# brendisurfs/Distributed-Backtesting-Exploration

Hardware: AMD Instinct MI355X
Metric: bar-evals/sec (symbols x params x bars) (higher is better)
Workload: dtype f64+int64; 1 GPU; BASELINE config 2: SMA fast/slow crossover, 5,000 symbols x 2,520 daily bars x 400 params per GPU; symbols_total=5000, symbols_per_gpu=5000, bars=2520, params=400, topk=100, parallelism=dp1 (contiguous symbol shards; exchange: none)

## Files before the change

### distributed-backtesting-exploration_amd/csrc/device_common.h

```cpp
#pragma once
#include <type_traits>

#include "internal.h"

namespace bt {

__host__ __device__ inline uint64_t trade_mix(uint64_t w) {
    const uint64_t z = (w ^ (w >> 29)) * 0xBF58476D1CE4E5B9ULL;
    return z ^ (z >> 32);
}
__host__ __device__ inline uint64_t trade_mix_et(uint32_t e, uint32_t t, bool lg) {
    const uint32_t lo = e ^ (t << 2) ^ (t << 31);
    const uint32_t hi = (t >> 1) ^ (lg ? 0x40000002u : 0u);
    const uint64_t z = (((uint64_t)hi << 32) | lo) * 0xBF58476D1CE4E5B9ULL;
    return z ^ (z >> 32);
}
constexpr int kDstLevels = 6;
constexpr int kKeyStride = kTile + 1;

typedef __int128 i128;
typedef __attribute__((address_space(3))) double lds_f64;

struct __attribute__((aligned(16))) Agg {
    int32_t mx, mn, dd, du;
// ... 22 lines not shown
}

__device__ __forceinline__ Agg dst_query(const Agg* D, const int32_t* cT, int a, int b) {
    if (a == b) return agg_one(cT[a]);
    const int r = dst_row(a, b);
    return agg_merge(D[r * kTile + a], D[r * kTile + b]);
}

__device__ __forceinline__ Agg dst_query_bf(const Agg* D, int a, int b) {
    const Agg* Dr = dst_rowp(D, a, b);
    return agg_merge(Dr[a], Dr[b]);
}

__device__ __forceinline__ Agg dst_query_w(const Agg* D, int a, int b) {
    const Agg* Dr = dst_rowp(D, a, b);
    const int4 u = *reinterpret_cast<const int4*>(Dr + a);
    const int4 v = *reinterpret_cast<const int4*>(Dr + b);
    asm volatile("" ::"v"(u.x), "v"(u.y), "v"(u.z), "v"(u.w), "v"(v.x), "v"(v.y), "v"(v.z), "v"(v.w));
    return agg_merge(Agg{u.x, u.y, u.z, u.w}, Agg{v.x, v.y, v.z, v.w});
}

constexpr Agg kAggId = {0, 0x7FFFFFFF, 0, 0};

__device__ __forceinline__ int64_t wave_iscan_i64(int64_t x) {
    uint32_t lo = (uint32_t)x, hi = (uint32_t)((uint64_t)x >> 32);
#define BT_DPP_STEP(ctrl, rmask)                                                      \
    {                                                                                 \
        const uint32_t ylo = __builtin_amdgcn_update_dpp(0u, lo, ctrl, rmask, 0xf, false); \
        const uint32_t yhi = __builtin_amdgcn_update_dpp(0u, hi, ctrl, rmask, 0xf, false); \
        const uint64_t r = (((uint64_t)hi << 32) | lo) + (((uint64_t)yhi << 32) | ylo);   \
        lo = (uint32_t)r;                                                             \
        hi = (uint32_t)(r >> 32);                                                     \
    }
    BT_DPP_STEP(0x111, 0xf)
    BT_DPP_STEP(0x112, 0xf)
    BT_DPP_STEP(0x114, 0xf)
    BT_DPP_STEP(0x118, 0xf)
    BT_DPP_STEP(0x142, 0xa)
    BT_DPP_STEP(0x143, 0xc)
#undef BT_DPP_STEP
    return (int64_t)(((uint64_t)hi << 32) | lo);
}

#define BT_S64_CTRLS(X)                                                                   \
    X("row_shr:1 row_mask:0xf bank_mask:0xf bound_ctrl:1")                                \
    X("row_shr:2 row_mask:0xf bank_mask:0xf bound_ctrl:1")                                \
    X("row_shr:4 row_mask:0xf bank_mask:0xf bound_ctrl:1")                                \
    X("row_shr:8 row_mask:0xf bank_mask:0xf bound_ctrl:1")                                \
    X("row_bcast:15 row_mask:0xa bank_mask:0xf")                                          \
    X("row_bcast:31 row_mask:0xc bank_mask:0xf")
__device__ __forceinline__ int64_t wave_iscan_i64_ac(int64_t x) {
    uint32_t lo = (uint32_t)x, hi = (uint32_t)((uint64_t)x >> 32);
#define BT_S64_ONE(ctrl)                                                                   \
    "s_nop 1\n"                                                                            \
    "v_add_co_u32_dpp %0, vcc, %0, %0 " ctrl "\n"                                          \
    "v_addc_co_u32_dpp %1, vcc, %1, %1, vcc " ctrl "\n"
    asm volatile(BT_S64_CTRLS(BT_S64_ONE) "s_nop 1" : "+v"(lo), "+v"(hi) : : "vcc");
#undef BT_S64_ONE
    return (int64_t)(((uint64_t)hi << 32) | lo);
}
__device__ __forceinline__ void wave_iscan2_i64_ac(int64_t& x, int64_t& y) {
    uint32_t xl = (uint32_t)x, xh = (uint32_t)((uint64_t)x >> 32);
    uint32_t yl = (uint32_t)y, yh = (uint32_t)((uint64_t)y >> 32);
#define BT_S64_TWO(ctrl)                                                                   \
    "v_add_co_u32_dpp %0, vcc, %0, %0 " ctrl "\n"                                          \
    "v_addc_co_u32_dpp %1, vcc, %1, %1, vcc " ctrl "\n"                                    \
    "v_add_co_u32_dpp %2, vcc, %2, %2 " ctrl "\n"                                          \
    "v_addc_co_u32_dpp %3, vcc, %3, %3, vcc " ctrl "\n"
    asm volatile("s_nop 1\n" BT_S64_CTRLS(BT_S64_TWO) "s_nop 1"
                 : "+v"(xl), "+v"(xh), "+v"(yl), "+v"(yh) : : "vcc");
#undef BT_S64_TWO
    x = (int64_t)(((uint64_t)xh << 32) | xl);
    y = (int64_t)(((uint64_t)yh << 32) | yl);
}
#undef BT_S64_CTRLS

__device__ __forceinline__ uint32_t wave_iscan_u32(uint32_t x) {
    x += __builtin_amdgcn_update_dpp(0u, x, 0x111, 0xf, 0xf, false);
    x += __builtin_amdgcn_update_dpp(0u, x, 0x112, 0xf, 0xf, false);
    x += __builtin_amdgcn_update_dpp(0u, x, 0x114, 0xf, 0xf, false);
    x += __builtin_amdgcn_update_dpp(0u, x, 0x118, 0xf, 0xf, false);
    x += __builtin_amdgcn_update_dpp(0u, x, 0x142, 0xa, 0xf, false);
    x += __builtin_amdgcn_update_dpp(0u, x, 0x143, 0xc, 0xf, false);
    return x;
}

template <int CTRL>
__device__ __forceinline__ int32_t dpp(int32_t old, int32_t x) {
    int32_t r = (int32_t)__builtin_amdgcn_update_dpp((uint32_t)old, (uint32_t)x, CTRL, 0xf, 0xf, false);
    asm volatile("" : "+v"(r));
    return r;
}

template <int M>
__device__ __forceinline__ int32_t dst_partner(int32_t x, int lane) {
    if constexpr (M == 1) {
        return dpp<0xB1>(0, x);
    } else if constexpr (M == 2) {
        return dpp<0x0F>(0, x);
    } else if constexpr (M == 3) {
        const int32_t hm = dpp<0x141>(0, x);
        const int32_t q3 = dpp<0xFF>(0, hm), q0 = dpp<0x00>(0, hm);
        return (lane & 4) ? q3 : q0;
    } else if constexpr (M == 4) {
        const int32_t r0 = dpp<0x150>(0, x), r15 = dpp<0x15F>(0, x);
        return (lane & 8) ? r0 : r15;
    } else {
        static_assert(M == 5, "six levels for 64-lane tiles");
        const int32_t l0 = (int32_t)__builtin_amdgcn_readlane((uint32_t)x, 0);
        const int32_t l31 = (int32_t)__builtin_amdgcn_readlane((uint32_t)x, 31);
        const int32_t l32 = (int32_t)__builtin_amdgcn_readlane((uint32_t)x, 32);
        const int32_t l63 = (int32_t)__builtin_amdgcn_readlane((uint32_t)x, 63);
        return (lane & 16) ? ((lane & 32) ? l32 : l0) : ((lane & 32) ? l63 : l31);
    }
}

template <int M, bool LDSX = false>
__device__ __forceinline__ Agg dst_partner_agg(const Agg& a, int lane) {
    if constexpr (LDSX && M >= 3) {
        constexpr int half = 1 << (M - 1), grp = 1 << M;
        const int src = (lane & half) ? (lane & ~(grp - 1)) : (lane | (grp - 1));
        return Agg{__builtin_amdgcn_ds_bpermute(src << 2, a.mx), __builtin_amdgcn_ds_bpermute(src << 2, a.mn),
                   __builtin_amdgcn_ds_bpermute(src << 2, a.dd), __builtin_amdgcn_ds_bpermute(src << 2, a.du)};
    }
    return Agg{dst_partner<M>(a.mx, lane), dst_partner<M>(a.mn, lane), dst_partner<M>(a.dd, lane),
               dst_partner<M>(a.du, lane)};
}

template <bool LDSX = false>
__device__ __forceinline__ void dst_build(int32_t c, int lane, Agg* D) {
    if (LDSX) asm volatile("" : "+v"(lane));
    Agg S = agg_one(c), Pp = S;
    D[(kDstLevels - 1) * kTile + lane] = S;
    auto level = [&](auto mtag) {
        constexpr int m = decltype(mtag)::value;
        const bool left = (lane & (1 << (m - 1))) == 0;
        const Agg part = dst_partner_agg<m, LDSX>(agg_sel(left, S, Pp), lane);
        S = agg_sel(left, agg_merge(S, part), S);
        Pp = agg_sel(left, Pp, agg_merge(part, Pp));
        D[(kDstLevels - 1 - m) * kTile + lane] = agg_sel(((lane >> m) & 1) != 0, Pp, S);
    };
    level(std::integral_constant<int, 1>{});
    level(std::integral_constant<int, 2>{});
    level(std::integral_constant<int, 3>{});
    level(std::integral_constant<int, 4>{});
    level(std::integral_constant<int, 5>{});
    static_assert(kDstLevels == 6, "levels 1..5 above");
}

__device__ __forceinline__ int64_t lane63_i64(int64_t x) {
    const uint32_t lo = __builtin_amdgcn_readlane((uint32_t)x, 63);
    const uint32_t hi = __builtin_amdgcn_readlane((uint32_t)((uint64_t)x >> 32), 63);
    return (int64_t)(((uint64_t)hi << 32) | lo);
}

__device__ __forceinline__ void fixed_ret(int32_t c, int32_t cp, int64_t& q, int64_t& q2) {
    const double ret = (double)((int64_t)c - cp) / (double)cp;
    q = (int64_t)rint(ret * 72057594037927936.0);
    const double rr = ret * ret;
    q2 = (int64_t)rint(rr * 72057594037927936.0);
}

__device__ __forceinline__ void wave_add_trades(const Out& out, int ntr) {
    unsigned long long v = (unsigned long long)ntr;
#pragma unroll
    for (int d = 32; d > 0; d >>= 1) v += __shfl_down(v, d, 64);
// ... 5 lines not shown
```

### distributed-backtesting-exploration_amd/csrc/engine.cpp

```cpp
#include <algorithm>
#include <cmath>
#include <cstdio>
#include <cstdlib>
#include <cstring>
#include <memory>
#include <string>
#include <vector>

#include "batch.h"
#include "csv.h"
#include "engine_state.h"
#include "topk_rules.h"

using namespace bt;

static thread_local std::string g_err;

void bt::set_last_error(const std::string& s) { g_err = s; }

namespace {

const char* kernel_name(int32_t strategy) {
    switch (strategy) {
        case BT_SMA_CROSS: return "bt::sma_kernel";
        case BT_EMA_OLS: return "bt::ema_tile_kernel";
        default: return "bt::boll_tile_kernel";
    }
}

std::string validate_and_copy(bt_engine* e, const bt_config& c) {
    const std::string err = plan_grid(c, e->grid);
    if (!err.empty()) return err;
    AxisSpec ax[4];
    const int nax = config_axes(c, ax);
    for (int i = 0; i < nax; ++i) e->ax[i].assign(ax[i].v, ax[i].v + ax[i].n);
    e->P = e->grid.n_params;
    if (c.annualization <= 0) return "annualization must be positive";
    e->grid.sqrt_ann = std::sqrt((double)c.annualization);
    if (c.topk < 0 || c.topk > kTopkMax) return "topk must be in [0, 1024]";
    if ((c.flags & BT_FLAG_PARITY) && c.trade_cap <= 0) return "parity mode needs trade_cap > 0";
    return "";
}

void upload_grid(bt_engine* e) {
    const int32_t** dst[4] = {&e->grid.a, &e->grid.b, &e->grid.c, &e->grid.d};
    for (int i = 0; i < 4; ++i) {
        *dst[i] = nullptr;
        if (e->ax[i].empty()) continue;
        e->d_axes[i].ensure(e->ax[i].size());
        HIPCHK(hipMemcpy(e->d_axes[i].p, e->ax[i].data(), e->ax[i].size() * 4, hipMemcpyHostToDevice));
        *dst[i] = e->d_axes[i].p;
    }
    e->grid.kwin = nullptr;
    e->grid.krecip = nullptr;
    if (e->cfg.strategy == BT_SMA_CROSS) {
        std::vector<int32_t> win(e->ax[0]);
        win.insert(win.end(), e->ax[1].begin(), e->ax[1].end());
        win.resize((win.size() + kKeyGrab - 1) / kKeyGrab * kKeyGrab, 1);
        std::vector<double> recip(win.size());
        for (size_t i = 0; i < win.size(); ++i) recip[i] = key_recip(win[i]);
        e->d_kwin.ensure(win.size());
        e->d_krecip.ensure(win.size());
        HIPCHK(hipMemcpy(e->d_kwin.p, win.data(), win.size() * sizeof(int32_t), hipMemcpyHostToDevice));
        HIPCHK(hipMemcpy(e->d_krecip.p, recip.data(), recip.size() * sizeof(double), hipMemcpyHostToDevice));
        e->grid.kwin = e->d_kwin.p;
        e->grid.krecip = e->d_krecip.p;
    }
}

static_assert(kStageAlign == kRowAlign, "batch.h lays staging rows out as the device columns");

void set_dataset(bt_engine* e, std::vector<SymDesc>&& syms, int64_t rows) {
    sync_all(e);
    e->syms = std::move(syms);
    e->rows = rows;
    e->max_bars = 0;
    for (const SymDesc& sd : e->syms) e->max_bars = std::max(e->max_bars, sd.bars);
    const size_t n_sym = e->syms.size();
    e->d_syms.ensure(std::max<size_t>(1, n_sym));
    if (n_sym)
        HIPCHK(hipMemcpyAsync(e->d_syms.p, e->syms.data(), n_sym * sizeof(SymDesc),
                              hipMemcpyHostToDevice, e->stream));
    const size_t r = std::max<int64_t>(1, rows);
    e->d_c.ensure(r);
    if (has_hl(e)) {
        e->d_h.ensure(r);
        e->d_l.ensure(r);
    }
    e->ran = false;
}

void layout(bt_engine* e, int32_t n_sym, const int32_t* bars, const int64_t* ids) {
    std::vector<SymDesc> syms((size_t)n_sym);
    int64_t off = 0;
    for (int32_t s = 0; s < n_sym; ++s) {
        syms[s].off = off;
        syms[s].bars = bars[s];
        syms[s].id = (int32_t)ids[s];
        off += align_rows(bars[s]);
    }
    set_dataset(e, std::move(syms), off);
}

TopkWork topk_work(bt_engine* e) {
    return TopkWork{e->d_hist.p, e->d_state.p, e->d_counts.p, e->d_above.p, e->d_cand.p,
                    kTopkCap, e->d_top.p + 1, reinterpret_cast<int32_t*>(e->d_top.p)};
}

void ensure_outputs(bt_engine* e) {
    const size_t n = (size_t)e->syms.size() * e->P;
    for (int b = 0; b < 2; ++b) {
        e->d_sum[b].ensure(std::max<size_t>(1, n));
        e->d_key[b].ensure(std::max<size_t>(1, n));
    }
    e->d_ntr_ring.ensure(kNtrRing);
    if (e->cfg.flags & BT_FLAG_PARITY) {
        e->d_sums.ensure(std::max<size_t>(1, n));
        e->d_trades.ensure(std::max<size_t>(1, n * (size_t)e->cfg.trade_cap));
    }
    if (e->cfg.topk > 0 && !e->topk_ready) {
        e->d_hist.ensure(4096);
        e->d_counts.ensure(2);
        e->d_state.ensure(4);
        e->d_above.ensure(kTopkCap);
        e->d_cand.ensure(kTopkCap);
        e->d_top.ensure(kTopkMax + 1);
        e->h_top.ensure(kTopkMax + 1);
        HIPCHK(launch_topk_init(topk_work(e), e->stream));
        e->topk_ready = true;
    }
}

void run_impl(bt_engine* e) {
    activate(e);
    ensure_outputs(e);
    const int32_t S = (int32_t)e->syms.size();
    const int64_t run = e->nrun++;
    const int b = (int)(run & 1);
    e->cur = b;
    if (e->tdone_armed[b] && hipEventQuery(e->ev_tdone[b]) != hipSuccess)
        HIPCHK(hipStreamWaitEvent(e->stream, e->ev_tdone[b], 0));
    Out out{};
    out.sum = e->d_sum[b].p;
    out.key = e->d_key[b].p;
    const bool parity = (e->cfg.flags & BT_FLAG_PARITY) != 0;
// ... 559 lines not shown
```

### distributed-backtesting-exploration_amd/csrc/internal.h

```cpp
#pragma once
#include <hip/hip_runtime.h>
#include <stdint.h>

#include <string>

#include "../../include/bt.h"

#ifdef BT_PROFILING
#define BT_ABL(g, bit) (((g).ablate & (bit)) != 0)
#define BT_PRIO(g, shift, dflt) (BT_ABL(g, 1 << 20) ? (((g).ablate >> (shift)) & 3) : (dflt))
#else
#define BT_ABL(g, bit) false
#define BT_PRIO(g, shift, dflt) (dflt)
#endif
constexpr int kDbgSlots = 80, kDbgBlocks = 1024;

namespace bt {

constexpr int kTile = 64;
constexpr int kRowAlign = 64;

struct SymDesc {
    int64_t off;
    int32_t bars;
    int32_t id;
};

struct Grid {
    int32_t strategy;
    int32_t n_params;
    int32_t na, nb, nc, nd;
    int32_t band_bps, k_den;
    int32_t wmax;
    int32_t ring;
    double sqrt_ann;
    double kn2[8];
    int32_t kmin_idx;
    int32_t ablate;
    const int32_t* a;
    const int32_t* b;
    const int32_t* c;
    const int32_t* d;
    const int32_t* kwin;
    const double* krecip;
};
constexpr int kKeyGrab = 4;

struct Out {
    bt_summary* sum;
    uint64_t* key;
    bt_sums* sums;
    bt_trade* trades;
    int32_t trade_cap;
    unsigned long long* n_trades;
    unsigned long long* dbg;
};

struct SegRec {
    int32_t ntr, expo;
    int32_t start_pos, start_e;
    int32_t end_pos, end_e, end_ce, pad;
    int32_t end_agg[4];
    int64_t R;
    int64_t A, B, C, D;
    uint64_t h;
    uint64_t s1lo;
    int64_t s1hi;
    uint64_t s2lo;
    int64_t s2hi;
};
static_assert(sizeof(SegRec) == 128, "SegRec layout");
struct SmaSegRec {
    int32_t ntr;
    int32_t e0;
    int32_t start_pos, end_pos;
    int32_t end_e, end_ce;
    int32_t x1, px1;
    int32_t agg1[4];
    int32_t end_agg[4];
    int64_t R;
    int64_t B, C, D;
    uint64_t h;
    uint64_t s1lo, s2lo;
    int32_t s1hi, s2hi;
};
static_assert(sizeof(SmaSegRec) == sizeof(SegRec), "SmaSegRec is one 128-B SegRec slot");
struct SegArgs {
    SegRec* rec;
    int8_t* pos;
    unsigned long long* refixed;
    double* ema;
    int32_t G;
    int32_t burn_tiles;
};
constexpr int kEmaSegStride = 128;
struct LaunchPlan;
hipError_t launch_gen(const SymDesc* syms, int32_t n_sym, uint64_t seed, int32_t freq,
                      int32_t* o, int32_t* h, int32_t* l, int32_t* c, hipStream_t st);
hipError_t launch_sma(const SymDesc* syms, int32_t n_sym, const int32_t* close, const Grid& g,
                      const Out& out, bool parity, const SegArgs& seg, const LaunchPlan& pl,
                      hipStream_t st);
hipError_t launch_ema_ols(const SymDesc* syms, int32_t n_sym, const int32_t* close, const Grid& g,
                          const Out& out, bool parity, const SegArgs& seg, const LaunchPlan& pl,
                          hipStream_t st);
hipError_t launch_boll(const SymDesc* syms, int32_t n_sym, const int32_t* high, const int32_t* low,
                       const int32_t* close, const Grid& g, const Out& out, bool parity,
                       const SegArgs& seg, const LaunchPlan& pl, hipStream_t st);

struct ReplayLane {
    int64_t off;
    int32_t bars;
    int32_t param;
};
struct ReplayOut {
    bt_summary* sum;
    bt_trade* trades;
    int32_t trade_cap;
    int64_t* equity;
    int8_t* pos;
    int64_t pitch;
};
hipError_t launch_replay(const ReplayLane* lanes, int32_t n, const int32_t* high, const int32_t* low,
                         const int32_t* close, const Grid& g, const ReplayOut& o, hipStream_t st);

struct WfArgs {
    const SymDesc* syms;
    const int32_t* bounds;
    bt_fold* rec;
    bt_wf_step* steps;
    int32_t n_rows, P, K;
    int32_t train, j0, n_steps;
};
struct WalkfwdPlan;
hipError_t launch_wf_walk(const WfArgs& a, const int32_t* high, const int32_t* low, const int32_t* close,
                          const Grid& g, hipStream_t st);
hipError_t launch_wf_select(const WfArgs& a, const Grid& g, const WalkfwdPlan& pl, hipStream_t st);

struct PfLane {
    int64_t off;
    int32_t bars;
    int32_t param;
    int32_t from, to;
};
static_assert(sizeof(PfLane) == 24, "PfLane layout");
struct PfWork {
    unsigned long long* acc_pnl;
    unsigned long long* acc_cnt;
    int64_t pitch;
    int32_t R;
    int32_t T;
    int32_t n_lanes, lo, hi;
    int64_t* pnl;
    int64_t* equity;
    int32_t* n_long;
    int32_t* n_short;
    bt_pf_summary* sum;
};
struct PortfolioPlan;
hipError_t launch_portfolio(const PfLane* lanes, int32_t n, const int32_t* high, const int32_t* low,
                            const int32_t* close, const Grid& g, const PfWork& w, const PortfolioPlan& pl,
                            hipStream_t st);

struct SurfacePlan;
struct SurfaceWork {
    bt_param_agg* partial;
    bt_param_agg* fold;
    bt_topk_rec* best_partial;
    bt_param_agg* agg;
    bt_topk_rec* best;
};
hipError_t launch_surface(const bt_summary* sum, const int32_t* ids, int32_t id_stride, int32_t S,
                          int32_t P, const SurfacePlan& pl, const SurfaceWork& w, hipStream_t st);

constexpr int kTopkCap = 2048;
constexpr int kTopkMax = 1024;
struct TopkWork {
    unsigned int* hist;
    unsigned long long* state;
    unsigned int* counts;
    unsigned long long* above;
    unsigned long long* cand;
    int cap;
    bt_topk_rec* out;
    int32_t* out_n;
};
hipError_t launch_topk(const uint64_t* key, const bt_summary* sum, const SymDesc* syms,
                       int64_t n, int32_t P, int32_t k, const TopkWork& w, hipStream_t st, bool lds_free_hist = false);
hipError_t launch_topk_init(const TopkWork& w, hipStream_t st);

void set_last_error(const std::string& s);
inline bool topk_less(const bt_topk_rec& a, const bt_topk_rec& b);
struct ExchangeView {
    hipStream_t tstream;
    int32_t device, topk;
    const bt_topk_rec* d_top;
    const unsigned long long* d_ntr;
    int64_t bar_evals;
};
bool engine_exchange_view(bt_engine* e, ExchangeView& v, std::string& err);
void engine_exchange_enqueued(bt_engine* e);

__host__ __device__ inline double key_recip(int W) { return (1.0 / (double)W) * (1.0 + 0x1p-47); }

__host__ __device__ inline uint64_t order_key(double x) {
    union { double d; uint64_t u; } v;
    v.d = x;
    return (v.u >> 63) ? ~v.u : (v.u | 0x8000000000000000ULL);
}

__host__ __device__ inline double i128_to_double(uint64_t lo, int64_t hi) {
    const bool neg = hi < 0;
    uint64_t mh = (uint64_t)hi, ml = lo;
    if (neg) {
        ml = ~ml + 1;
        mh = ~mh + (ml == 0 ? 1 : 0);
    }
    if (mh == 0 && ml == 0) return 0.0;
    int lz = mh ? __builtin_clzll(mh) : 64 + __builtin_clzll(ml);
    uint64_t nh, nl;
    if (lz >= 64) {
        nh = ml << (lz - 64);
        nl = 0;
    } else if (lz == 0) {
        nh = mh;
        nl = ml;
    } else {
        nh = (mh << lz) | (ml >> (64 - lz));
        nl = ml << lz;
    }
    uint64_t mant = nh >> 11;
    const uint64_t rem_hi = nh & 0x7FFULL;
    const uint64_t half = 0x400ULL;
    bool up;
    if (rem_hi > half) up = true;
    else if (rem_hi < half) up = false;
    else up = (nl != 0) || (mant & 1);
    mant += up ? 1 : 0;
    double r = (double)mant;
#ifdef __HIP_DEVICE_COMPILE__
    r = ldexp(r, 75 - lz);
#else
    r = __builtin_ldexp(r, 75 - lz);
#endif
    return neg ? -r : r;
}

inline bool topk_less(const bt_topk_rec& a, const bt_topk_rec& b) {
    const uint64_t ka = order_key(a.sharpe), kb = order_key(b.sharpe);
    if (ka != kb) return ka > kb;
    if (a.sym != b.sym) return a.sym < b.sym;
    return a.param < b.param;
}

__host__ __device__ inline double sharpe_fx(uint64_t s1lo, int64_t s1hi, uint64_t s2lo,
                                            int64_t s2hi, int32_t bars, double sqrt_ann) {
    if (bars < 2) return 0.0;
    const double n = (double)(bars - 1);
    const double m = ldexp(i128_to_double(s1lo, s1hi), -56) / n;
    const double mm = m * m;
    const double v = ldexp(i128_to_double(s2lo, s2hi), -56) / n - mm;
    return v > 0 ? (m / sqrt(v)) * sqrt_ann : 0.0;
}

__host__ __device__ inline double sharpe_ticks(uint64_t s1lo, int64_t s1hi, uint64_t s2lo,
                                               int64_t s2hi, int32_t n_bars, double sqrt_ann) {
    if (n_bars < 1) return 0.0;
    const double n = (double)n_bars;
    const double m = i128_to_double(s1lo, s1hi) / n;
    const double mm = m * m;
    const double v = i128_to_double(s2lo, s2hi) / n - mm;
    return v > 0 ? (m / sqrt(v)) * sqrt_ann : 0.0;
}

}
```

### distributed-backtesting-exploration_amd/csrc/k_sma.hip

```cpp
#include <algorithm>
#include <cmath>
#include <cstdlib>

#include "launch_run.h"
#include "lds_layout.h"
#include "plan.h"
#include "tile_common.h"

namespace bt {

namespace {

constexpr int kCmpDepth1 = 2;

struct ScanCarry {
    int64_t P;
    int32_t prevc;
    uint32_t tv;
};

__device__ __forceinline__ int32_t load_close(const int32_t* __restrict__ crow, int B, int t) {
    return t < B ? crow[t] : 0;
}

__device__ __forceinline__ void ring_store(double* ring, int R, int t0, int lane, double v) {
    const int i = (t0 + lane + 1) & (R - 1);
    ring[i] = v;
    const int rb = t0 & (R - 1);
    if (rb == 0 || rb == R - kTile) {
        if (i < kRingMirror) ring[R + i] = v;
    }
}

__device__ __forceinline__ void stage_ring(int32_t c, int B, int t0, int lane, int R, double* ring,
                                           int32_t* cT, int64_t* ql, int32_t* narrow,
                                           ScanCarry& cy) {
    const int t = t0 + lane;
    const bool valid = t < B;
    const int32_t cp = (int32_t)__builtin_amdgcn_update_dpp((uint32_t)cy.prevc, (uint32_t)c,
                                                            0x138, 0xf, 0xf, false);
    const int64_t inc = wave_iscan_i64((int64_t)c);
    ring_store(ring, R, t0, lane, (double)(cy.P + inc));
    cT[lane] = c;
    int64_t q = 0, q2 = 0;
    uint32_t dv = 0;
    if (valid && t >= 1) {
        fixed_ret(c, cp, q, q2);
        dv = (uint32_t)abs(c - cp);
    }
    ql[lane] = wave_iscan_i64(q);
    ql[kTile + lane] = wave_iscan_i64(q2);
    const bool big = __ballot(dv >= (1u << 25)) != 0;
    const uint32_t tvt = __builtin_amdgcn_readlane(wave_iscan_u32(min(dv, 1u << 25)), 63);
    cy.tv = big ? (1u << 31) : min(cy.tv + tvt, 1u << 31);
    if (lane == 0) *narrow = cy.tv < (1u << 30);
    cy.P += lane63_i64(inc);
    cy.prevc = (int32_t)__builtin_amdgcn_readlane((uint32_t)c, 63);
}


__device__ __forceinline__ int32_t floor_key(double F, double iw) {
    return (int32_t)(F * iw);
}

__host__ __device__ inline uint32_t key_round_len(int nwp, int nwaves) {
    return (uint32_t)kKeyGrab * ((uint32_t)nwp / kKeyGrab + 1 + (uint32_t)nwaves);
}

struct KeyGroup {
    int32_t W[kKeyGrab];
    double I[kKeyGrab];
};
typedef __attribute__((address_space(4))) const int32_t const_i32;
typedef __attribute__((address_space(4))) const double const_f64;
__device__ __forceinline__ KeyGroup key_group(const int32_t* kwin, const double* krecip,
                                              uint32_t w, int nwp) {
    const uint32_t i = min(w - (uint32_t)kKeyGrab, (uint32_t)(nwp - kKeyGrab));
    const_i32* cw = (const_i32*)kwin + i;
    const_f64* cr = (const_f64*)krecip + i;
    KeyGroup g;
#pragma unroll
    for (int q = 0; q < kKeyGrab; ++q) {
        g.W[q] = cw[q];
        g.I[q] = cr[q];
    }
    return g;
}

__device__ __forceinline__ void stage_keys(int t0, int B, int nwp, int nf, int wmax, int R,
                                           const double* ring, const int32_t* __restrict__ kwin,
                                           const double* __restrict__ krecip, int32_t* K,
                                           uint32_t* ctr, uint32_t round, int nwaves, int lane,
                                           const int32_t* cTr, Agg* Dr) {
    const int t = t0 + lane;
    const double* ringl = ring + lane;
    const double top = ringl[(t0 + 1) & (R - 1)];
    const bool full = t0 + 1 - wmax >= 0 && t0 + kTile <= B;
    const uint32_t base = round * key_round_len(nwp, nwaves);
    uint32_t w = __builtin_amdgcn_readlane(grab_issue<kKeyGrab>(ctr, lane), 0) - base;
    KeyGroup gw = key_group(kwin, krecip, w, nwp);
#pragma unroll 1
    while (w < (uint32_t)(nwp + kKeyGrab)) {
        const uint32_t vn = grab_issue<kKeyGrab>(ctr, lane);
        if (w == 0) {
            dst_build<true>(cTr[lane], lane, Dr);
            w = __builtin_amdgcn_readlane(vn, 0) - base;
            gw = key_group(kwin, krecip, w, nwp);
            continue;
        }
        w -= kKeyGrab;
        int32_t kq[kKeyGrab];
#pragma unroll
        for (int q = 0; q < kKeyGrab; ++q) {
            const double F = top - ringl[(t0 + 1 - gw.W[q]) & (R - 1)];
            kq[q] = floor_key(F, gw.I[q]);
        }
        int32_t* Kw = K + w * kKS + lane;
        if (full) {
#pragma unroll
            for (int q = 0; q < kKeyGrab; ++q) Kw[q * kKS] = kq[q];
        } else {
            const bool tin = t < B;
#pragma unroll
            for (int q = 0; q < kKeyGrab; ++q)
                Kw[q * kKS] = (tin && t + 1 - gw.W[q] >= 0) ? kq[q] : ((int)(w + q) < nf ? -1 : -2);
        }
        w = __builtin_amdgcn_readlane(vn, 0) - base;
        gw = key_group(kwin, krecip, w, nwp);
    }
}

__device__ __forceinline__ void cmp4(uint32_t& l, uint32_t& z, const int4& x, const int4& y) {
    const uint32_t d0 = (uint32_t)(x.x - y.x), d1 = (uint32_t)(x.y - y.y);
    const uint32_t d2 = (uint32_t)(x.z - y.z), d3 = (uint32_t)(x.w - y.w);
    l = __builtin_amdgcn_alignbit(l, d0, 31);
    l = __builtin_amdgcn_alignbit(l, d1, 31);
    l = __builtin_amdgcn_alignbit(l, d2, 31);
    l = __builtin_amdgcn_alignbit(l, d3, 31);
    z = min(min(z, d0), d1);
    z = min(min(z, d2), d3);
}

__device__ __forceinline__ void eq4(uint32_t& e, const int4& x, const int4& y) {
    e = __builtin_amdgcn_alignbit(e, min((uint32_t)(x.x - y.x), 1u) - 1u, 31);
    e = __builtin_amdgcn_alignbit(e, min((uint32_t)(x.y - y.y), 1u) - 1u, 31);
    e = __builtin_amdgcn_alignbit(e, min((uint32_t)(x.z - y.z), 1u) - 1u, 31);
    e = __builtin_amdgcn_alignbit(e, min((uint32_t)(x.w - y.w), 1u) - 1u, 31);
}
__device__ __forceinline__ uint64_t eq_word(const int32_t* k1, const int32_t* k2) {
    const int4* r1 = reinterpret_cast<const int4*>(k1);
    const int4* r2 = reinterpret_cast<const int4*>(k2);
    uint32_t e0 = 0, e1 = 0;
#pragma unroll 1
    for (int v = 0; v < 8; ++v) {
        eq4(e0, r1[v], r2[v]);
        eq4(e1, r1[v + 8], r2[v + 8]);
    }
    return ((uint64_t)__builtin_bitreverse32(e1) << 32) | __builtin_bitreverse32(e0);
}

}

struct SmaAcct {
    int32_t pos, e, ce, sb, ntr, e0;
    int32_t g32, m32, r32;
    int64_t R, gap, mdd;
    uint64_t ps1, ps2, h;
    I96 s1, s2;
    Agg agg;
    int64_t Bq, C, D;
    int32_t carried, x1, px1;
    Agg agg1;
};


template <bool PARITY, bool MERGE = true, bool SEG = false, bool NARROW = false>
__device__ __forceinline__ void sma_close(SmaAcct& a, const Agg& seg, int t, int32_t cx,
// ... 50 lines not shown
    if (RESET_AGG) a.agg = kAggId;
    a.pos = np;
}

template <bool PARITY, bool ONE_TRIP, bool FIRST, bool SEG, bool NARROW>
__device__ __forceinline__ void sma_reverse(SmaAcct& a, uint64_t& F, uint64_t& alt, int t0,
                                            const int32_t* cT, const int64_t* ql, const Agg* D,
                                            bt_trade* tr, int cap) {
    const int b = __builtin_ctzll(F);
    F &= F - 1;
    Agg seg;
    int32_t cx;
    uint64_t qb;
    if (ONE_TRIP) {
        const Agg* Dr = dst_rowp(D, a.sb, b);
        const Agg d1 = Dr[a.sb], d2 = Dr[b];
        cx = cT[b];
        qb = (uint64_t)ql[b];
        asm volatile("" ::"v"(d1.mx), "v"(d1.mn), "v"(d1.dd), "v"(d1.du), "v"(d2.mx),
                     "v"(d2.mn), "v"(d2.dd), "v"(d2.du), "v"(cx), "v"((uint32_t)qb),
                     "v"((uint32_t)(qb >> 32)));
        seg = agg_merge(d1, d2);
    } else {
        seg = dst_query_bf(D, a.sb, b);
        cx = cT[b];
        qb = (uint64_t)ql[b];
    }
    alt = qb - alt;
    sma_close<PARITY, FIRST, SEG, NARROW>(a, seg, t0 + b, cx, tr, cap);
    sma_open<FIRST>(a, b, t0 + b, cx, -a.pos);
}

template <bool PARITY, bool ONE_TRIP, bool SEG, bool NARROW>
__device__ __forceinline__ void sma_flips(SmaAcct& a, uint64_t F, int t0, int bl, uint64_t LONG,
                                          const int32_t* cT, const int64_t* ql, const Agg* D,
                                          bt_trade* tr, int cap) {
    const uint64_t FX = (bl >= 0 && bl < 64) ? (F & (1ULL << bl)) : 0ULL;
    F ^= FX;
    if (a.pos == 0 && F != 0) {
        const int b = __builtin_ctzll(F);
        F &= F - 1;
        const int np = ((LONG >> b) & 1) ? 1 : -1;
        const uint64_t qx = (uint64_t)ql[b];
        a.ps1 += np > 0 ? (uint64_t)0 - qx : qx;
        a.ps2 -= (uint64_t)ql[kTile + b];
        a.e0 = t0 + b;
        sma_open(a, b, t0 + b, cT[b], np);
    }
    uint64_t alt = 0;
    if (F) sma_reverse<PARITY, ONE_TRIP, true, SEG, NARROW>(a, F, alt, t0, cT, ql, D, tr, cap);
    while (F) sma_reverse<PARITY, ONE_TRIP, false, SEG, NARROW>(a, F, alt, t0, cT, ql, D, tr, cap);
    a.ps1 += a.pos > 0 ? (uint64_t)0 - (alt << 1) : alt << 1;
    if (FX) {
        const int b = bl;
        const uint64_t qx = (uint64_t)ql[b];
        sma_close<PARITY, true, SEG, NARROW>(a, dst_query_bf(D, a.sb, b), t0 + b, cT[b], tr, cap);
        a.ps1 += a.pos > 0 ? qx : (uint64_t)0 - qx;
        a.ps2 += (uint64_t)ql[kTile + b];
        a.pos = 0;
    }
}

template <bool PARITY, bool STAMPS, bool ONE_TRIP, bool SEG>
__device__ __forceinline__ void sma_body(const SymDesc* __restrict__ syms,
                                         const int32_t* __restrict__ close, const Grid& g,
                                         const Out& out, int dedicated, const SegArgs& sg,
                                         int fix_seg) {
    extern __shared__ __attribute__((aligned(16))) unsigned char smem[];
    const int nf = g.na, ns = g.nb, nw = nf + ns;
    const int R = g.ring;
    const SmaLds LL = sma_lds_layout(R, nw);
    double* ring = reinterpret_cast<double*>(smem + LL.ring);
    int32_t* keys = reinterpret_cast<int32_t*>(smem + LL.keys);
    Agg* dst = reinterpret_cast<Agg*>(smem + LL.dst);
    int32_t* cts = reinterpret_cast<int32_t*>(smem + LL.ct);
    int64_t* qls = reinterpret_cast<int64_t*>(smem + LL.ql);
    int32_t* nars = reinterpret_cast<int32_t*>(smem + LL.nar);
    uint32_t* ctr = reinterpret_cast<uint32_t*>(smem + LL.ctr);

    const int tid = threadIdx.x;
    const int lane = tid & 63;
    const int wave = __builtin_amdgcn_readfirstlane(tid >> 6);
    const int nwaves = (int)blockDim.x >> 6;
    const bool helper = (tid >> 6) == nwaves - 1;
    const int nparam_threads = dedicated ? (int)blockDim.x - 64 : (int)blockDim.x;
    const SymDesc sd = syms[blockIdx.x];
    const int B = sd.bars;
    const int ntiles = (B + kTile - 1) / kTile;
    const int P = g.n_params;
    const int j = blockIdx.y * nparam_threads + tid;
    const bool active = tid < nparam_threads && j < P;
    const int kf = active ? j % nf : 0;
    const int ks = nf + (active ? j / nf : 0);
    const int p = (kf * ns) + (ks - nf);
    const int32_t* crow = close + sd.off;

    SegRange sr{0, 0, 0, 0, ntiles};
    SmaSegRec* mine = nullptr;
    size_t ipos = 0, npos = 0;
    if (SEG) {
        sr = seg_range(sg, fix_seg, ntiles, g.wmax);
        const size_t per_seg = (size_t)gridDim.x * P;
        ipos = sr.seg * per_seg + (size_t)blockIdx.x * P + p;
        npos = (size_t)sg.G * per_seg;
        mine = reinterpret_cast<SmaSegRec*>(sg.rec) + ipos;
        if (fix_seg > 0) {
            if (!__syncthreads_or(active && sg.pos[ipos] != sg.pos[npos + ipos - per_seg])) return;
            if (tid == 0) atomicAdd(sg.refixed, 1ULL);
        }
    }
    const int T_scan = sr.T_scan, T_walk = sr.T_walk, T_acct = sr.T_acct, T_end = sr.T_end;

    const int nwp = (nw + kKeyGrab - 1) / kKeyGrab * kKeyGrab;
    const uint32_t key_round = key_round_len(nwp, nwaves);
    if (tid == 0) {
        const int i0 = (T_scan * kTile) & (R - 1);
        ring[i0] = 0.0;
        if (i0 == 0) ring[R] = 0.0;
        *ctr = (uint32_t)T_walk * key_round;
    }
    __syncthreads();
    const int32_t wf = g.kwin[kf], ws = g.kwin[ks];
    const int warm = max(wf, ws) - 1;
    const uint32_t fsw = (uint32_t)wf | ((uint32_t)ws << 16);
    int wmin = active ? warm : 0x7fffffff;
#pragma unroll
    for (int o = 32; o > 0; o >>= 1) wmin = min(wmin, __shfl_xor(wmin, o));
    const int kfirst = __builtin_amdgcn_readfirstlane(wmin) >> 6;

    ScanCarry cy{0, (T_scan > 0 && T_scan * kTile - 1 < B) ? crow[T_scan * kTile - 1] : 0};
    if (SEG && helper && T_scan < T_walk) {
        constexpr int kLookAhead = 8;
        int32_t cn[kLookAhead];
#pragma unroll
        for (int u = 0; u < kLookAhead; ++u) cn[u] = load_close(crow, B, (T_scan + u) * kTile + lane);
#pragma unroll 1
        for (int T0 = T_scan; T0 < T_walk; T0 += kLookAhead) {
#pragma unroll
            for (int u = 0; u < kLookAhead; ++u) {
                const int T = T0 + u;
                if (T < T_walk) {
                    const int32_t c = cn[u];
                    cn[u] = load_close(crow, B, (T + kLookAhead) * kTile + lane);
                    const int64_t inc = wave_iscan_i64((int64_t)c);
                    ring[(T * kTile + lane + 1) & (R - 1)] = (double)(cy.P + inc);
                    cy.P += lane63_i64(inc);
                    cy.prevc = (int32_t)__builtin_amdgcn_readlane((uint32_t)c, 63);
                }
            }
        }
        ring[R + lane] = ring[lane];
    }
    int32_t cpre = 0;
    if (helper) {
        const int b0 = T_walk * kTile;
        const int32_t c0 = load_close(crow, B, b0 + lane), c1 = load_close(crow, B, b0 + kTile + lane);
        cpre = load_close(crow, B, b0 + 2 * kTile + lane);
        const int s0 = T_walk % kStages, s1 = (T_walk + 1) % kStages;
        if (T_walk < T_end) stage_ring(c0, B, b0, lane, R, ring, cts + s0 * kTile, qls + s0 * 2 * kTile, nars + s0, cy);
        __syncthreads();
        if (T_walk + 1 < T_end)
            stage_ring(c1, B, b0 + kTile, lane, R, ring, cts + s1 * kTile, qls + s1 * 2 * kTile, nars + s1, cy);
    } else {
        __syncthreads();
    }
    if (T_walk < T_end)
        stage_keys(T_walk * kTile, B, nwp, nf, g.wmax, R, ring, g.kwin, g.krecip,
                   keys + (T_walk & 1) * nwp * kKS, ctr, (uint32_t)T_walk, nwaves, lane,
                   cts + (T_walk % kStages) * kTile, dst + (T_walk % kDstStages) * kDstLevels * kTile);
    __syncthreads();

    SmaAcct a;
    a.pos = a.e = a.ce = a.sb = a.ntr = a.e0 = 0;
    a.g32 = a.m32 = a.r32 = 0;
    a.R = a.gap = a.mdd = 0;
    a.ps1 = a.ps2 = 0;
    a.h = 0;
    a.s1.clear();
    a.s2.clear();
    a.agg = kAggId;
    a.Bq = a.C = a.D = kNegInf;
    a.carried = a.x1 = a.px1 = 0;
    a.agg1 = kAggId;
    int32_t start_pos = 0;
    if (SEG && fix_seg > 0 && active) a.pos = sg.pos[npos + ipos - (size_t)gridDim.x * P];
    auto enter_acct = [&]() {
        start_pos = a.pos;
        a.carried = a.pos != 0;
        a.agg = kAggId;
        a.sb = 0;
        a.R = 0;
        a.Bq = a.C = a.D = kNegInf;
        a.ntr = 0;
        a.h = 0;
        a.s1.clear();
        a.s2.clear();
        a.ps1 = a.ps2 = 0;
        a.e0 = -1;
        a.x1 = -1;
        a.px1 = 0;
        a.agg1 = kAggId;
    };
    if (SEG && T_walk == T_acct) enter_acct();
    bt_trade* tr = nullptr;
    auto result_index = [&]() -> size_t {
        int le = lane;
        asm volatile("" : "+v"(le));
        const int je = blockIdx.y * nparam_threads + wave * 64 + le;
        return (size_t)blockIdx.x * P + (size_t)((je % nf) * ns + je / nf);
    };
    const size_t gi = (size_t)blockIdx.x * P + p;
    if (PARITY && active) tr = out.trades + gi * out.trade_cap;
    const int cap = out.trade_cap;

    constexpr bool stamps = STAMPS;
    uint64_t st_acc[7] = {0, 0, 0, 0, 0, 0, 0};
    uint64_t st_prev = 0;
#define BT_STAMP(i)                                             \
    if (stamps) {                                               \
        const uint64_t now_ = __builtin_amdgcn_s_memtime();     \
        st_acc[i] += now_ - st_prev;                            \
        st_prev = now_;                                         \
    }
    if (stamps) st_prev = __builtin_amdgcn_s_memtime();

    auto tile_step = [&](auto narrow_tag, const int k) __attribute__((always_inline)) {
        constexpr bool NARROW = decltype(narrow_tag)::value;
        const int t0 = k * kTile;
        if (helper && k + 2 < T_end && !BT_ABL(g, 1)) {
            if (!BT_ABL(g, 32)) __builtin_amdgcn_s_setprio(2);
            const int s = (k + 2) % kStages;
            stage_ring(cpre, B, t0 + 2 * kTile, lane, R, ring, cts + s * kTile,
                       qls + s * 2 * kTile, nars + s, cy);
            cpre = load_close(crow, B, t0 + 3 * kTile + lane);
            __builtin_amdgcn_s_setprio(0);
        }
        BT_STAMP(0)
        if (SEG && active && k == T_acct && k != T_walk) enter_acct();
        if (active && k >= kfirst) {
            if (ONE_TRIP) __builtin_amdgcn_s_setprio(1);
            const int s = k % kStages;
            const int32_t* cT = cts + s * kTile;
            const int64_t* ql = qls + s * 2 * kTile;
            const Agg* D = dst + (k % kDstStages) * kDstLevels * kTile;
            const int32_t* K = keys + (k & 1) * nwp * kKS;
            const int4* k1 = reinterpret_cast<const int4*>(K + kf * kKS);
            const int4* k2 = reinterpret_cast<const int4*>(K + ks * kKS);
            uint32_t l0 = 0, l1 = 0, z = ~0u;
            if (!BT_ABL(g, 4)) {
#pragma unroll
                for (int v = 0; v < 16; ++v) {
                    if (v < 8) cmp4(l0, z, k1[v], k2[v]);
                    else cmp4(l1, z, k1[v], k2[v]);
                    if (ONE_TRIP ? ((v % kCmpDepth1) == kCmpDepth1 - 1) : (v & 1))
                        __builtin_amdgcn_sched_barrier(0);
                }
            }
            BT_STAMP(2)
            uint64_t L = ((uint64_t)__builtin_bitreverse32(l1) << 32) | __builtin_bitreverse32(l0);
            const int lastdec = B - 2 - t0;
            const int wb = warm - t0;
            const int bl = B - 1 - t0;
            uint64_t LONG, F;
            if (z != 0 && wb <= 0 && lastdec >= 63) {
                LONG = ~L;
                F = (LONG ^ ((LONG << 1) | (uint64_t)(a.pos == 1))) | (uint64_t)(a.pos == 0);
            } else {
                uint64_t vm = lastdec >= 63 ? ~0ULL : (lastdec < 0 ? 0ULL : ((1ULL << (lastdec + 1)) - 1));
                vm &= wb <= 0 ? ~0ULL : (wb >= 64 ? 0ULL : (~0ULL << wb));
                uint64_t G, T = 0;
                if (z != 0) {
                    G = ~L & vm;
                } else {
                    const uint64_t E = eq_word(K + kf * kKS, K + ks * kKS);
                    G = ~(L | E) & vm;
                    T = E & vm;
                }
                L &= vm;
                while (T) {
                    const int b = __builtin_ctzll(T);
                    T &= T - 1;
                    const int t = t0 + b;
                    const double top = ring[(t + 1) & (R - 1)];
                    const int fw = (int)(fsw & 0xffffu), sw = (int)(fsw >> 16);
                    const int64_t Fs = (int64_t)(top - ring[(t + 1 - fw) & (R - 1)]) * sw;
                    const int64_t Lf = (int64_t)(top - ring[(t + 1 - sw) & (R - 1)]) * fw;
                    G |= (uint64_t)(Fs > Lf) << b;
                    L |= (uint64_t)(Fs < Lf) << b;
                }
                uint64_t SHORT;
                {
                    const uint64_t A = ~L;
                    const uint64_t s1 = A + G;
                    uint64_t cout = s1 < A;
                    const uint64_t sum = s1 + (uint64_t)(a.pos == 1);
                    cout |= sum < s1;
                    LONG = ((sum ^ A ^ G) >> 1) | (cout << 63);
                }
                {
                    const uint64_t A = ~G;
                    const uint64_t s1 = A + L;
                    uint64_t cout = s1 < A;
                    const uint64_t sum = s1 + (uint64_t)(a.pos == -1);
                    cout |= sum < s1;
                    SHORT = ((sum ^ A ^ L) >> 1) | (cout << 63);
                }
                if (bl < 64) {
                    const uint64_t keep = bl <= 0 ? 0ULL : ((1ULL << bl) - 1);
                    LONG &= keep;
                    SHORT &= keep;
                }
                const uint64_t pL = (LONG << 1) | (uint64_t)(a.pos == 1);
                const uint64_t pS = (SHORT << 1) | (uint64_t)(a.pos == -1);
                F = (LONG ^ pL) | (SHORT ^ pS);
            }
            BT_STAMP(3)
            uint64_t Fw = F;
            if (BT_ABL(g, 8)) {
                asm volatile("" ::"v"((uint32_t)Fw), "v"((uint32_t)(Fw >> 32)));
                Fw = 0;
            }
            sma_flips<PARITY, ONE_TRIP, SEG, NARROW>(a, Fw, t0, bl, LONG, cT, ql, D, tr, cap);
            BT_STAMP(4)
            if (a.pos != 0) {
                a.agg = agg_merge(a.agg, dst_query_bf(D, a.sb, kTile - 1));
                a.sb = 0;
                const uint64_t q63 = (uint64_t)ql[kTile - 1];
                a.ps1 += a.pos > 0 ? q63 : (uint64_t)0 - q63;
                a.ps2 += (uint64_t)ql[2 * kTile - 1];
            }
            if ((k & 1) || k + 1 == T_end) {
                a.s1.add((int64_t)a.ps1);
                a.s2.add((int64_t)a.ps2);
                a.ps1 = a.ps2 = 0;
            }
            BT_STAMP(5)
            if (ONE_TRIP) __builtin_amdgcn_s_setprio(0);
        }
        if (k + 1 < T_end && !BT_ABL(g, 2))
            stage_keys(t0 + kTile, B, nwp, nf, g.wmax, R, ring, g.kwin, g.krecip, keys + ((k + 1) & 1) * nwp * kKS,
                       ctr, (uint32_t)(k + 1), nwaves, lane, cts + ((k + 1) % kStages) * kTile,
                       dst + ((k + 1) % kDstStages) * kDstLevels * kTile);
        BT_STAMP(1)
        __syncthreads();
        BT_STAMP(6)
    };
    int k = T_walk;
    if (!SEG && k < T_end) {
        bool nar = __builtin_amdgcn_readfirstlane(nars[k % kStages]) != 0;
        while (nar) {
            const int32_t nn = k + 1 < T_end ? nars[(k + 1) % kStages] : 0;
            tile_step(std::true_type{}, k);
            nar = __builtin_amdgcn_readfirstlane(nn) != 0;
            ++k;
        }
        a.gap = (uint32_t)a.g32;
        a.mdd = (uint32_t)a.m32;
        a.R = a.r32;
    }
    for (; k < T_end; ++k) tile_step(std::false_type{}, k);
#undef BT_STAMP
    if (stamps && lane == 0) {
        unsigned long long* d = out.dbg + (helper ? 8 : 0);
        for (int i = 0; i < 7; ++i) atomicAdd(&d[i], (unsigned long long)st_acc[i]);
        atomicAdd(&d[7], 1ULL);
    }
    if (SEG) {
        if (active) {
            SmaSegRec r;
            r.ntr = a.ntr;
            r.e0 = a.e0;
            r.start_pos = start_pos;
            r.end_pos = a.pos;
            r.end_e = a.carried ? -1 : a.e;
            r.end_ce = a.ce;
            r.x1 = a.x1;
            r.px1 = a.px1;
            const Agg g1 = a.x1 >= 0 ? a.agg1 : a.agg;
            r.agg1[0] = g1.mx;
            r.agg1[1] = g1.mn;
            r.agg1[2] = g1.dd;
            r.agg1[3] = g1.du;
            r.end_agg[0] = a.agg.mx;
            r.end_agg[1] = a.agg.mn;
            r.end_agg[2] = a.agg.dd;
            r.end_agg[3] = a.agg.du;
            r.R = a.R;
            r.B = a.Bq;
            r.C = a.C;
            r.D = a.D;
            r.h = a.h;
            r.s1lo = a.s1.lo;
            r.s1hi = a.s1.hi;
            r.s2lo = a.s2.lo;
            r.s2hi = a.s2.hi;
            *mine = r;
            sg.pos[ipos] = (int8_t)start_pos;
            sg.pos[npos + ipos] = (int8_t)a.pos;
        }
        return;
    }
    if (active) {
        const uint64_t s1lo = a.s1.lo, s2lo = a.s2.lo;
        const int64_t s1hi = a.s1.hi64(), s2hi = a.s2.hi64();
        const double sh = sharpe_fx(s1lo, s1hi, s2lo, s2hi, B, g.sqrt_ann);
        bt_summary r;
        r.n_trades = a.ntr;
        r.status = 0;
        r.pnl = a.R;
        r.mdd = a.mdd;
        r.exposure = a.ntr > 0 ? B - 1 - a.e0 : 0;
        r.sharpe = sh;
        r.hash = a.h;
        const size_t go = result_index();
        out.sum[go] = r;
        out.key[go] = order_key(sh);
        if (out.sums != nullptr) out.sums[go] = bt_sums{s1lo, s1hi, s2lo, s2hi};
    }
    wave_add_trades(out, active ? a.ntr : 0);
}

template <bool PARITY, bool STAMPS, bool ONE_TRIP>
__global__ __launch_bounds__(1024) __attribute__((amdgpu_waves_per_eu(6))) void sma_kernel(
    const SymDesc* __restrict__ syms, const int32_t* __restrict__ close, Grid g, Out out,
    int dedicated) {
    sma_body<PARITY, STAMPS, ONE_TRIP, false>(syms, close, g, out, dedicated, SegArgs{}, 0);
}

template <bool ONE_TRIP>
__global__ __launch_bounds__(1024) void sma_seg_kernel(const SymDesc* __restrict__ syms,
                                                       const int32_t* __restrict__ close, Grid g,
                                                       Out out, int dedicated, SegArgs sg,
                                                       int fix_seg) {
    sma_body<false, false, ONE_TRIP, true>(syms, close, g, out, dedicated, sg, fix_seg);
}

// ... 105 lines not shown
```

Baseline: 4748 billion bar-evals/s.

## Scale SMA key reciprocals by running close-price magnitude via precomputed power-of-two tables

The helper wave now tracks a running maximum of close prices and packs a shift amount, derived from its leading zeros, into the per-stage narrow flag word. Key staging uses that shift to pick one of 31 precomputed reciprocal tables scaled by powers of two. The goal is to keep key quantities in a better-conditioned range, presumably so cheaper or narrower comparisons can be used downstream. It adds a max-scan per tile and a 31x larger reciprocal table, and it changes how the stage word is encoded and read.

```diff
diff --git a/distributed-backtesting-exploration_amd/csrc/device_common.h b/distributed-backtesting-exploration_amd/csrc/device_common.h
--- a/distributed-backtesting-exploration_amd/csrc/device_common.h
+++ b/distributed-backtesting-exploration_amd/csrc/device_common.h
@@ -128,6 +128,16 @@
     x += __builtin_amdgcn_update_dpp(0u, x, 0x118, 0xf, 0xf, false);
     x += __builtin_amdgcn_update_dpp(0u, x, 0x142, 0xa, 0xf, false);
     x += __builtin_amdgcn_update_dpp(0u, x, 0x143, 0xc, 0xf, false);
+    return x;
+}
+
+__device__ __forceinline__ uint32_t wave_maxscan_u32(uint32_t x) {
+    x = max(x, (uint32_t)__builtin_amdgcn_update_dpp(0u, x, 0x111, 0xf, 0xf, false));
+    x = max(x, (uint32_t)__builtin_amdgcn_update_dpp(0u, x, 0x112, 0xf, 0xf, false));
+    x = max(x, (uint32_t)__builtin_amdgcn_update_dpp(0u, x, 0x114, 0xf, 0xf, false));
+    x = max(x, (uint32_t)__builtin_amdgcn_update_dpp(0u, x, 0x118, 0xf, 0xf, false));
+    x = max(x, (uint32_t)__builtin_amdgcn_update_dpp(0u, x, 0x142, 0xa, 0xf, false));
+    x = max(x, (uint32_t)__builtin_amdgcn_update_dpp(0u, x, 0x143, 0xc, 0xf, false));
     return x;
 }
 
diff --git a/distributed-backtesting-exploration_amd/csrc/engine.cpp b/distributed-backtesting-exploration_amd/csrc/engine.cpp
--- a/distributed-backtesting-exploration_amd/csrc/engine.cpp
+++ b/distributed-backtesting-exploration_amd/csrc/engine.cpp
@@ -57,10 +57,12 @@
         std::vector<int32_t> win(e->ax[0]);
         win.insert(win.end(), e->ax[1].begin(), e->ax[1].end());
         win.resize((win.size() + kKeyGrab - 1) / kKeyGrab * kKeyGrab, 1);
-        std::vector<double> recip(win.size());
-        for (size_t i = 0; i < win.size(); ++i) recip[i] = key_recip(win[i]);
+        const size_t nwp = win.size();
+        std::vector<double> recip(kKeyScales * nwp);
+        for (int s = 0; s < kKeyScales; ++s)
+            for (size_t i = 0; i < nwp; ++i) recip[s * nwp + i] = std::ldexp(key_recip(win[i]), s);
         e->d_kwin.ensure(win.size());
-        e->d_krecip.ensure(win.size());
+        e->d_krecip.ensure(recip.size());
         HIPCHK(hipMemcpy(e->d_kwin.p, win.data(), win.size() * sizeof(int32_t), hipMemcpyHostToDevice));
         HIPCHK(hipMemcpy(e->d_krecip.p, recip.data(), recip.size() * sizeof(double), hipMemcpyHostToDevice));
         e->grid.kwin = e->d_kwin.p;
diff --git a/distributed-backtesting-exploration_amd/csrc/internal.h b/distributed-backtesting-exploration_amd/csrc/internal.h
--- a/distributed-backtesting-exploration_amd/csrc/internal.h
+++ b/distributed-backtesting-exploration_amd/csrc/internal.h
@@ -45,6 +45,7 @@
     const double* krecip;
 };
 constexpr int kKeyGrab = 4;
+constexpr int kKeyScales = 31;
 
 struct Out {
     bt_summary* sum;
@@ -201,6 +202,10 @@
 void engine_exchange_enqueued(bt_engine* e);
 
 __host__ __device__ inline double key_recip(int W) { return (1.0 / (double)W) * (1.0 + 0x1p-47); }
+__host__ __device__ inline int key_shift(uint32_t cmax) {
+    const int lz = cmax ? __builtin_clz(cmax) : 32;
+    return lz < 1 ? 0 : (lz > kKeyScales ? kKeyScales - 1 : lz - 1);
+}
 
 __host__ __device__ inline uint64_t order_key(double x) {
     union { double d; uint64_t u; } v;
diff --git a/distributed-backtesting-exploration_amd/csrc/k_sma.hip b/distributed-backtesting-exploration_amd/csrc/k_sma.hip
--- a/distributed-backtesting-exploration_amd/csrc/k_sma.hip
+++ b/distributed-backtesting-exploration_amd/csrc/k_sma.hip
@@ -17,7 +17,14 @@
     int64_t P;
     int32_t prevc;
     uint32_t tv;
+    uint32_t cmax;
 };
+
+__device__ __forceinline__ int32_t stage_word(bool narrow, int shift) {
+    return (int32_t)narrow | (shift << 1);
+}
+__device__ __forceinline__ bool stage_narrow(int32_t w) { return (w & 1) != 0; }
+__device__ __forceinline__ int stage_shift(int32_t w) { return w >> 1; }
 
 __device__ __forceinline__ int32_t load_close(const int32_t* __restrict__ crow, int B, int t) {
     return t < B ? crow[t] : 0;
@@ -33,7 +40,7 @@
 }
 
 __device__ __forceinline__ void stage_ring(int32_t c, int B, int t0, int lane, int R, double* ring,
-                                           int32_t* cT, int64_t* ql, int32_t* narrow,
+                                           int32_t* cT, int64_t* ql, int32_t* word,
                                            ScanCarry& cy) {
     const int t = t0 + lane;
     const bool valid = t < B;
@@ -53,7 +60,8 @@
     const bool big = __ballot(dv >= (1u << 25)) != 0;
     const uint32_t tvt = __builtin_amdgcn_readlane(wave_iscan_u32(min(dv, 1u << 25)), 63);
     cy.tv = big ? (1u << 31) : min(cy.tv + tvt, 1u << 31);
-    if (lane == 0) *narrow = cy.tv < (1u << 30);
+    cy.cmax = max(cy.cmax, __builtin_amdgcn_readlane(wave_maxscan_u32((uint32_t)c), 63));
+    if (lane == 0) *word = stage_word(cy.tv < (1u << 30), key_shift(cy.cmax));
     cy.P += lane63_i64(inc);
     cy.prevc = (int32_t)__builtin_amdgcn_readlane((uint32_t)c, 63);
 }
@@ -91,8 +99,9 @@
                                            const double* ring, const int32_t* __restrict__ kwin,
                                            const double* __restrict__ krecip, int32_t* K,
                                            uint32_t* ctr, uint32_t round, int nwaves, int lane,
-                                           const int32_t* cTr, Agg* Dr) {
+                                           const int32_t* cTr, Agg* Dr, int32_t sw) {
     const int t = t0 + lane;
+    krecip += stage_shift(__builtin_amdgcn_readfirstlane(sw)) * nwp;
     const double* ringl = ring + lane;
     const double top = ringl[(t0 + 1) & (R - 1)];
     const bool full = t0 + 1 - wmax >= 0 && t0 + kTile <= B;
@@ -309,7 +318,7 @@
     const int lane = tid & 63;
     const int wave = __builtin_amdgcn_readfirstlane(tid >> 6);
     const int nwaves = (int)blockDim.x >> 6;
-    const bool helper = (tid >> 6) == nwaves - 1;
+    const bool helper = wave == nwaves - 1;
     const int nparam_threads = dedicated ? (int)blockDim.x - 64 : (int)blockDim.x;
     const SymDesc sd = syms[blockIdx.x];
     const int B = sd.bars;
@@ -359,6 +368,7 @@
     if (SEG && helper && T_scan < T_walk) {
         constexpr int kLookAhead = 8;
         int32_t cn[kLookAhead];
+        uint32_t vmax = 0;
 #pragma unroll
         for (int u = 0; u < kLookAhead; ++u) cn[u] = load_close(crow, B, (T_scan + u) * kTile + lane);
 #pragma unroll 1
@@ -368,6 +378,7 @@
                 const int T = T0 + u;
                 if (T < T_walk) {
                     const int32_t c = cn[u];
+                    vmax = max(vmax, (uint32_t)c);
                     cn[u] = load_close(crow, B, (T + kLookAhead) * kTile + lane);
                     const int64_t inc = wave_iscan_i64((int64_t)c);
                     ring[(T * kTile + lane + 1) & (R - 1)] = (double)(cy.P + inc);
@@ -377,6 +388,7 @@
             }
         }
         ring[R + lane] = ring[lane];
+        cy.cmax = __builtin_amdgcn_readlane(wave_maxscan_u32(vmax), 63);
     }
     int32_t cpre = 0;
     if (helper) {
@@ -394,7 +406,8 @@
     if (T_walk < T_end)
         stage_keys(T_walk * kTile, B, nwp, nf, g.wmax, R, ring, g.kwin, g.krecip,
                    keys + (T_walk & 1) * nwp * kKS, ctr, (uint32_t)T_walk, nwaves, lane,
-                   cts + (T_walk % kStages) * kTile, dst + (T_walk % kDstStages) * kDstLevels * kTile);
+                   cts + (T_walk % kStages) * kTile, dst + (T_walk % kDstStages) * kDstLevels * kTile,
+                   nars[T_walk % kStages]);
     __syncthreads();
 
     SmaAcct a;
@@ -454,6 +467,7 @@
     auto tile_step = [&](auto narrow_tag, const int k) __attribute__((always_inline)) {
         constexpr bool NARROW = decltype(narrow_tag)::value;
         const int t0 = k * kTile;
+        int32_t nn = (!SEG && k + 1 < T_end) ? nars[(k + 1) % kStages] : 0;
         if (helper && k + 2 < T_end && !BT_ABL(g, 1)) {
             if (!BT_ABL(g, 32)) __builtin_amdgcn_s_setprio(2);
             const int s = (k + 2) % kStages;
@@ -564,21 +578,21 @@
             BT_STAMP(5)
             if (ONE_TRIP) __builtin_amdgcn_s_setprio(0);
         }
+        if (SEG && k + 1 < T_end) nn = nars[(k + 1) % kStages];
         if (k + 1 < T_end && !BT_ABL(g, 2))
             stage_keys(t0 + kTile, B, nwp, nf, g.wmax, R, ring, g.kwin, g.krecip, keys + ((k + 1) & 1) * nwp * kKS,
                        ctr, (uint32_t)(k + 1), nwaves, lane, cts + ((k + 1) % kStages) * kTile,
-                       dst + ((k + 1) % kDstStages) * kDstLevels * kTile);
+                       dst + ((k + 1) % kDstStages) * kDstLevels * kTile, nn);
         BT_STAMP(1)
         __syncthreads();
         BT_STAMP(6)
+        return nn;
     };
     int k = T_walk;
     if (!SEG && k < T_end) {
-        bool nar = __builtin_amdgcn_readfirstlane(nars[k % kStages]) != 0;
+        bool nar = stage_narrow(__builtin_amdgcn_readfirstlane(nars[k % kStages]));
         while (nar) {
-            const int32_t nn = k + 1 < T_end ? nars[(k + 1) % kStages] : 0;
-            tile_step(std::true_type{}, k);
-            nar = __builtin_amdgcn_readfirstlane(nn) != 0;
+            nar = stage_narrow(__builtin_amdgcn_readfirstlane(tile_step(std::true_type{}, k)));
             ++k;
         }
         a.gap = (uint32_t)a.g32;
```

After: 4711 billion bar-evals/s. No clear change (-0.8%).
